# RohanVKashyap/resolution-pde

Measured on AMD Instinct MI355X. Metric: training samples/sec, FFNO2D NS 256^2, higher is better.
Workload: dtype f32; 1 GPU; FFNO2D(1,1,width=64,n_layers=4,n_modes=20,factor=4,ff_weight_norm,n_ff_layers=3,layer_norm,dropout=0.1) train step on [B,1,256,256] Gaussian random fields (BASELINE configs[2]); batch_per_gpu=32, global_batch=32, optimizer=AdamW lr=1e-3 (rpde.optim.FlatAdamW: torch.optim.AdamW's rule, one kernel), parallelism=single, grad_bucket_bytes=6828576, target=input advanced by a fixed spectral filter (utils/synthetic.py:advance)

## Files before the change

include/rpde.h:

```cpp
#ifndef RPDE_H
#define RPDE_H

#include <stddef.h>
#include <stdint.h>

#ifdef __cplusplus
extern "C" {
#endif

typedef enum {
  RPDE_OK = 0,
  RPDE_ERR_ARG = -1,
  RPDE_ERR_HIP = -2,
  RPDE_ERR_WORKSPACE = -3,
  RPDE_ERR_MODES = -4
} rpde_status;

enum { RPDE_NORM_BACKWARD = 0, RPDE_NORM_ORTHO = 1, RPDE_NORM_FORWARD = 2 };
enum { RPDE_MODE_FULL = 0, RPDE_MODE_LOWPASS = 1 };
enum { RPDE_ACT_IDENTITY = 0, RPDE_ACT_GELU = 1, RPDE_ACT_RELU = 2 };
enum { RPDE_EPI_MULAUX = 100 };

const char* rpde_last_error(void);
int rpde_version(void);
// ... 44 lines not shown
int rpde_fspectral1d_bwd(const float* grad_out, const float* spec_in, const float* w,
                         float* grad_x, float* grad_w, const float* grad_skip,
                         int B, int n, int C, int K, int mode, int norm,
                         void* ws, size_t ws_bytes, void* stream);

size_t rpde_fspectral2d_ws_bytes(int B, int M, int N, int C, int K);
size_t rpde_fspectral2d_spec_elems(int B, int M, int N, int C, int K, int axis );
int rpde_fspectral2d_fwd(const float* x, const float* w_y, const float* w_x, float* out,
                         float* spec_y, float* spec_x,
                         int B, int M, int N, int C, int K, int mode,
                         void* ws, size_t ws_bytes, void* stream);
int rpde_fspectral2d_bwd(const float* grad_out, const float* spec_y, const float* spec_x,
                         const float* w_y, const float* w_x,
                         float* grad_x, float* grad_wy, float* grad_wx, const float* grad_skip,
                         int B, int M, int N, int C, int K, int mode,
                         void* ws, size_t ws_bytes, void* stream);
size_t rpde_fspectral2d_prep_bytes(int M, int N, int C, int K);
size_t rpde_fspectral2d_eval_ws_bytes(int B, int M, int N, int C, int K);
int rpde_fspectral2d_prepare(const float* w_y, const float* w_x, int M, int N, int C, int K,
                             void* prep, size_t prep_bytes, void* stream);
int rpde_fspectral2d_fwd_prepared(const float* x, const void* prep, float* out, int B, int M, int N, int C, int K,
                                  void* ws, size_t ws_bytes, void* stream);

size_t rpde_spectral1d_ws_bytes(int B, int Cin, int Cout, int n, int K);
int rpde_spectral1d_fwd(const float* x, const float* w, float* out, float* spec_in,
                        int B, int Cin, int Cout, int n, int K, int act_in,
                        void* ws, size_t ws_bytes, void* stream);
int rpde_spectral1d_bwd(const float* grad_out, const float* spec_in, const float* w,
                        const float* x, float* grad_x, float* grad_w,
                        int B, int Cin, int Cout, int n, int K, int act_in,
                        void* ws, size_t ws_bytes, void* stream);

size_t rpde_spectral2d_ws_bytes(int B, int Cin, int Cout, int M, int N, int m1, int m2);
size_t rpde_spectral2d_spec_elems(int B, int Cin, int M, int N, int m1, int m2);
int rpde_spectral2d_fwd(const float* x, const float* w1, const float* w2, float* out, float* spec_in,
                        int B, int Cin, int Cout, int M, int N, int m1, int m2, int act_in,
                        void* ws, size_t ws_bytes, void* stream);
int rpde_spectral2d_bwd(const float* grad_out, const float* spec_in, const float* w1, const float* w2,
                        const float* x, float* grad_x, float* grad_w1, float* grad_w2,
                        int B, int Cin, int Cout, int M, int N, int m1, int m2, int act_in,
                        void* ws, size_t ws_bytes, void* stream);

typedef struct {
  int n_layers; int dim; int factor;
  int layer_norm; float ln_eps;
  float dropout_p; uint64_t seed;
// ... 266 lines not shown
```

resolution-pde_amd/csrc/ff_fused.hip:

```cpp
#include "ff_fused.h"
#include "cw.h"
#include "h2.h"
#include "pointwise.h"

namespace rpde {

#ifdef RPDE_STAMPS
__device__ unsigned long long g_ffstamps[3 * 64];
#define FFSTAMP(i) do { if (stamp_on && stamp_t < 8) g_ffstamps[stamp_w * 64 + stamp_t * 8 + (i)] = __builtin_amdgcn_s_memtime(); } while (0)
__device__ unsigned long long g_fbstamps[3 * 64];
#define FBSTAMP(i) do { if (stamp_on && stamp_t >= 0 && stamp_t < 8) g_fbstamps[stamp_w * 64 + stamp_t * 8 + (i)] = __builtin_amdgcn_s_memtime(); } while (0)
#else
#define FFSTAMP(i) do { } while (0)
#define FBSTAMP(i) do { } while (0)
#endif

constexpr int FF_WAVES = 8;
constexpr int FF_FRAGS = 24;
constexpr int FF_IMG_BYTES = FF_WAVES * FF_FRAGS * 2048;
constexpr int FF_NCONST = 16;
constexpr int FF_PREP_BLOCKS = FF_WAVES * FF_FRAGS * 64 / 1024;

__global__ __launch_bounds__(1024) void k_ff3_prep(const float* __restrict__ w1, const float* __restrict__ w2,
                                                   const float* __restrict__ w3, const float* __restrict__ b1,
// ... 394 lines not shown
    for (int k = 0; k < 64; ++k) wv2[k] = w2[(64 * part + k) * 256 + col];
#pragma unroll
    for (int k = 0; k < 64; ++k) b += fabsf(wv2[k]);
    colp[0][part][col] = a; colp[1][part][col] = b;
    __syncthreads();
    if (tid < 256) {
      r3 = (colp[0][0][tid] + colp[0][1][tid]) + (colp[0][2][tid] + colp[0][3][tid]);
      r2 = (colp[1][0][tid] + colp[1][1][tid]) + (colp[1][2][tid] + colp[1][3][tid]);
    }
  }
  float v[5] = {m1, m2, m3, r3, r2};
#pragma unroll
  for (int k = 0; k < 5; ++k) { v[k] = wave_max(v[k]); if (l == 0) red[k][wv] = v[k]; }
  __syncthreads();
  if (tid < 5) { float a = 0.f; for (int i = 0; i < 16; ++i) a = fmaxf(a, red[tid][i]); fin[tid] = a; }
  __syncthreads();
  float sc[3], iv[3];
#pragma unroll
  for (int k = 0; k < 3; ++k) h2_scale(fin[k], 0, sc[k], iv[k]);
  if (tid == 0 && blockIdx.x == 0) { consts[0] = iv[0]; consts[1] = iv[1]; consts[2] = iv[2]; consts[3] = fin[3]; consts[4] = fin[4]; }
  for (int it = blockIdx.x * 1024 + tid; it < FF_WAVES * FF_FRAGS * 64; it += gridDim.x * 1024) {
    const int ln = it & 63, f = (it >> 6) % FF_FRAGS, w = it / (64 * FF_FRAGS);
    const int g = ln >> 4, li = ln & 15;
    float x[8];
    if (f < 4) {
      const int hid = 16 * (2 * w + (f >> 1)) + li;
#pragma unroll
      for (int j = 0; j < 8; ++j) x[j] = w3[(32 * (f & 1) + frag_perm(g, j)) * 256 + hid] * sc[2];
    } else if (f < 20) {
      const int hid1 = 16 * (2 * w + ((f - 4) >> 3)) + li, kap = (f - 4) & 7;
#pragma unroll
      for (int j = 0; j < 8; ++j) x[j] = w2[(32 * kap + frag_perm(g, j)) * 256 + hid1] * sc[1];
    } else {
      const int feat = 16 * (f - 20) + li;
#pragma unroll
      for (int j = 0; j < 8; ++j) x[j] = w1[(32 * w + frag_perm(g, j)) * 64 + feat] * sc[0];
    }
    h2_put_frag(img + ((long)(w * FF_FRAGS + f)) * 2048 + ln * 16, x);
  }
}

constexpr int FFB_PART = 704;
struct FF3B {
  const float* g; const float* z3; const float* d1; const float* d2;
  float* dz3; float* du2; float* du1; float* dx;
  const char* wimg; const float* consts;
  const float* gamma; const float* beta;
  float* part;
  long P; int layer_norm; float eps; int post_act;
  DropCfg drop2;
  DropCfg drop0, drop1;
  float dmax;
  int ntiles;
};

constexpr int FB_DZBUF = 0;
constexpr int FB_DUBUF = FB_DZBUF + 8192;
constexpr int FB_W3L = FB_DUBUF + 32768;
constexpr int FB_D2 = FB_W3L + 32768;
// ... 410 lines not shown
```

resolution-pde_amd/csrc/fspectral.hip:

```cpp
#include "rpde_internal.h"
#include "plan.h"
#include "pointwise.h"
#include "fused_spectral.h"
#include "mix1d.h"

namespace rpde {

struct Axis {
  int n;
  int keff, kp;
  int rows;
  int zdiv;
  long s1, s2;
  long ld;
  const rpde_plan* plan;
};

static inline int split_for(long k_total, int tiles) {
  long s = 512 / (tiles > 0 ? tiles : 1);
  const long cap = (k_total + 127) / 128;
  if (s > cap) s = cap;
  if (s < 1) s = 1;
  if (s > 512) s = 512;
  return (int)s;
}

static int dft_analysis(const Axis& ax, const float* field, float* spec, int C, bool adjoint_of_synthesis, hipStream_t st) {
// ... 297 lines not shown
  RPDE_CARVE("fspectral1d_fwd", AxisFwdWork, wk, ws, ws_bytes, ax, C, mode, mix1d_ok(B, C));
  hipStream_t st = as_stream(stream);
  RPDE_TRY(make_axis(ax, n, K, norm, B, 1, (long)n * C, 0, C, st));
  return axis_fwd(ax, x, w, K, out, spec_in, C, mode, 0, wk, st);
}

int rpde_fspectral1d_bwd(const float* grad_out, const float* spec_in, const float* w, float* grad_x, float* grad_w,
                         const float* grad_skip, int B, int n, int C, int K, int mode, int norm, void* ws, size_t ws_bytes,
                         void* stream) {
  RPDE_CHECK_ARG(grad_out && spec_in && B > 0 && n > 0 && C > 0 && K > 0, "fspectral1d_bwd: bad arguments");
  RPDE_CHECK_ARG(mode == RPDE_MODE_LOWPASS || w, "fspectral1d_bwd: null weight");
  Axis ax; axis_dims(ax, n, K, B);
  RPDE_CARVE("fspectral1d_bwd", AxisBwdWork, wk, ws, ws_bytes, ax, C, mode, mix1d_ok(B, C));
  hipStream_t st = as_stream(stream);
  RPDE_TRY(make_axis(ax, n, K, norm, B, 1, (long)n * C, 0, C, st));
  return axis_bwd(ax, grad_out, spec_in, w, K, grad_x, grad_w, C, mode, 0, wk, st, grad_skip);
}

size_t rpde_fspectral2d_ws_bytes(int B, int M, int N, int C, int K) {
  Axis ay, ax;
  axes2d_dims(ay, ax, B, M, N, K);
  const size_t n = ws_max(axis_ws_bytes(ay, C), axis_ws_bytes(ax, C));
  if (!fused2d_ok(M, N, C, ay.keff, ax.keff)) return n;
  return ws_max(n, ws_max(ws_measure<Fused2dFwdWork>(ay, ax, C), ws_measure<Fused2dBwdWork>(ay, ax, C)));
}
size_t rpde_fspectral2d_spec_elems(int B, int M, int N, int C, int K, int axis) {
  Axis ay, ax;
  axes2d_dims(ay, ax, B, M, N, K);
  const Axis& a = axis == 0 ? ay : ax;
  return spec_floats(a, C) + (fused2d_ok(M, N, C, ay.keff, ax.keff) ? (size_t)a.rows : 0);
}

int rpde_fspectral2d_fwd(const float* x, const float* w_y, const float* w_x, float* out, float* spec_y, float* spec_x, int B,
                         int M, int N, int C, int K, int mode, void* ws, size_t ws_bytes, void* stream) {
  RPDE_CHECK_ARG(x && out && spec_y && spec_x && B > 0 && M > 0 && N > 0 && C > 0 && K > 0, "fspectral2d_fwd: bad arguments");
  RPDE_CHECK_ARG(mode == RPDE_MODE_LOWPASS || (w_y && w_x), "fspectral2d_fwd: null weight");
  RPDE_CHECK_ARG(mode == RPDE_MODE_FULL || mode == RPDE_MODE_LOWPASS, "fspectral2d_fwd: mode %d", mode);
  hipStream_t st = as_stream(stream);
  Axis ay, ax;
  axes2d_dims(ay, ax, B, M, N, K);
  Arena ar(ws, ws_bytes);
  if (fused2d_ok(M, N, C, ay.keff, ax.keff)) {
    const Fused2dFwdWork wk(ar, ay, ax, C);
    RPDE_CLAIM_WS("fspectral2d_fwd", ar, ws_bytes);
    RPDE_TRY(make_axes2d(ay, ax, B, M, N, C, K, st));
    return fused2d_fwd(ay, ax, x, w_y, w_x, out, spec_y, spec_x, B, M, N, C, K, mode, wk, st);
  }
// ... 77 lines not shown
```

resolution-pde_amd/models/ffno.py:

```python
from __future__ import annotations

import numpy as np
import torch
import torch.nn as nn

from models.custom_layer import WNLinear
from models.spectral_convolution import FSpectralConv1d, FSpectralConv2d
from rpde import ops


def _coord(c, device):
    if not isinstance(c, torch.Tensor):
        c = torch.tensor(c, dtype=torch.float)
    return c.to(device=device, dtype=torch.float32).contiguous()


class FFNO1D(nn.Module):
    def __init__(self, in_channels, out_channels, width=64, n_layers=4, n_modes=16, factor=4, ff_weight_norm=False,
                 n_ff_layers=2, layer_norm=False, dropout=0.0, grid=None, mode="full", fft_norm="ortho",
                 activation="identity", use_grid=True):
        super().__init__()
        self.in_channels, self.out_channels, self.hidden_dim = in_channels, out_channels, width
        self.n_layers, self.n_modes, self.grid = n_layers, n_modes, grid
        self.use_grid = grid
# ... 33 lines not shown
        self.fourier_layers = nn.ModuleList([
            FSpectralConv2d(width, n_modes, factor=factor, ff_weight_norm=ff_weight_norm, n_ff_layers=n_ff_layers,
                            layer_norm=layer_norm, dropout=dropout, mode=mode)
            for _ in range(n_layers)])
        self.out_proj = WNLinear(width, out_channels, wnorm=True) if ff_weight_norm else nn.Linear(width, out_channels)

    def get_grid(self, shape, device):
        b, m, n = shape[0], shape[1], shape[2]
        if self.grid is not None:
            gx, gy = _coord(self.grid[0], device), _coord(self.grid[1], device)
        else:
            gx = torch.tensor(np.linspace(0, 1, m), dtype=torch.float).to(device)
            gy = torch.tensor(np.linspace(0, 1, n), dtype=torch.float).to(device)
        gx = gx.reshape(1, m, 1, 1).repeat([b, 1, n, 1])
        gy = gy.reshape(1, 1, n, 1).repeat([b, m, 1, 1])
        return torch.cat((gx, gy), dim=-1)

    @staticmethod
    def _apply_linear(mod, h):
        if isinstance(mod, WNLinear):
            return mod(h)
        return ops.linear(h, mod.weight, mod.bias)

    def forward(self, x):
        if self.use_grid:
            gx = gy = None
            if self.grid is not None:
                gx, gy = _coord(self.grid[0], x.device), _coord(self.grid[1], x.device)
            h = ops.concat_grid(x, 2, 0.0, 1.0, channels_last=True, gridx=gx, gridy=gy)
        else:
            h = ops.to_channels_last(x)
        h = self._apply_linear(self.in_proj, h)
        for layer in self.fourier_layers:
            h, _ = layer(h, residual=h)
        return ops.to_channels_first(self._apply_linear(self.out_proj, h))
```

resolution-pde_amd/models/spectral_convolution.py:

```python
from __future__ import annotations

import torch
import torch.nn as nn
from torch.nn import functional as F

from models.custom_layer import FeedForward
from rpde import ops

act_registry = {"gelu": F.gelu, "identity": nn.Identity(), "relu": F.relu}


class SpectralConv1d(nn.Module):

    def __init__(self, in_channels, out_channels, modes1):
        super().__init__()
        self.in_channels, self.out_channels, self.modes1 = in_channels, out_channels, modes1
        self.scale = 1 / (in_channels * out_channels)
        self.weights1 = nn.Parameter(self.scale * torch.rand(in_channels, out_channels, modes1, dtype=torch.cfloat))

    def forward(self, x, act_in="identity"):
        return ops.spectral1d(x, self.weights1, act_in)


class SpectralConv2d(nn.Module):
# ... 46 lines not shown
        return self.backcast_ff(x, residual=residual, post_act=self.activation), None


class FSpectralConv2d(nn.Module):

    def __init__(self, d_model, modes, forecast_ff=None, backcast_ff=None, fourier_weight=None, factor=4,
                 ff_weight_norm=False, n_ff_layers=2, layer_norm=False, use_fork=False, dropout=0.0, mode="full"):
        super().__init__()
        self.in_dim = self.out_dim = d_model
        self.n_modes, self.mode, self.use_fork = modes, mode, use_fork
        self.fourier_weight = fourier_weight if fourier_weight else _fourier_weights(d_model, modes, 2)
        self.backcast_ff = backcast_ff if backcast_ff else FeedForward(
            d_model, factor, n_layers=n_ff_layers, ff_weight_norm=ff_weight_norm, layer_norm=layer_norm, dropout=dropout)
        self.forecast_ff = forecast_ff
        if use_fork and not self.forecast_ff:
            self.forecast_ff = FeedForward(
                d_model, factor, n_layers=n_ff_layers, ff_weight_norm=ff_weight_norm, layer_norm=layer_norm,
                dropout=dropout)

    def forward_fourier(self, x, with_skip=False):
        return ops.fspectral2d(x, self.fourier_weight[0], self.fourier_weight[1], self.n_modes, self.mode,
                               with_skip=with_skip)

    def forward(self, x, batch_dt=None, residual=None):
        if self.mode != "no-fourier":
            if residual is x and torch.is_grad_enabled() and x.requires_grad:
                x, residual = self.forward_fourier(x, with_skip=True)
            else:
                x = self.forward_fourier(x)
        b = self.backcast_ff(x, residual=residual)
        f = self.forecast_ff(x) if self.use_fork else None
        return b, f
```

resolution-pde_amd/rpde/_lib.py:

```python
from __future__ import annotations

import ctypes as C
import os
from typing import Optional, Sequence

import torch

_HERE = os.path.dirname(os.path.abspath(__file__))
LIB_PATH = os.environ.get("RPDE_LIB") or os.path.join(_HERE, "lib", "librpde_hip.so")

ACT = {"identity": 0, "gelu": 1, "relu": 2}
NORM = {"backward": 0, "ortho": 1, "forward": 2}
MODE = {"full": 0, "low-pass": 1}

ERR_ARG, ERR_HIP, ERR_WORKSPACE, ERR_MODES = -1, -2, -3, -4


class RpdeError(RuntimeError):
    pass


class GemmDesc(C.Structure):
    _fields_ = [
        ("A", C.c_void_p), ("B", C.c_void_p), ("C", C.c_void_p),
# ... 44 lines not shown
    "rpde_split_weights": (_I, [_P, _I, C.c_int64, _I, _I, _P, _P]),
    "rpde_fspectral1d_ws_bytes": (_Z, [_I, _I, _I, _I]),
    "rpde_fspectral1d_spec_elems": (_Z, [_I, _I, _I, _I]),
    "rpde_fspectral1d_fwd": (_I, [_P, _P, _P, _P, _I, _I, _I, _I, _I, _I, _P, _Z, _P]),
    "rpde_fspectral1d_bwd": (_I, [_P, _P, _P, _P, _P, _P, _I, _I, _I, _I, _I, _I, _P, _Z, _P]),
    "rpde_fspectral2d_ws_bytes": (_Z, [_I, _I, _I, _I, _I]),
    "rpde_fspectral2d_spec_elems": (_Z, [_I, _I, _I, _I, _I, _I]),
    "rpde_fspectral2d_fwd": (_I, [_P, _P, _P, _P, _P, _P, _I, _I, _I, _I, _I, _I, _P, _Z, _P]),
    "rpde_fspectral2d_bwd": (_I, [_P, _P, _P, _P, _P, _P, _P, _P, _P, _I, _I, _I, _I, _I, _I, _P, _Z, _P]),
    "rpde_spectral1d_ws_bytes": (_Z, [_I, _I, _I, _I, _I]),
    "rpde_spectral1d_fwd": (_I, [_P, _P, _P, _P, _I, _I, _I, _I, _I, _I, _P, _Z, _P]),
    "rpde_spectral1d_bwd": (_I, [_P, _P, _P, _P, _P, _P, _I, _I, _I, _I, _I, _I, _P, _Z, _P]),
    "rpde_spectral2d_ws_bytes": (_Z, [_I, _I, _I, _I, _I, _I, _I]),
    "rpde_spectral2d_spec_elems": (_Z, [_I, _I, _I, _I, _I, _I]),
    "rpde_spectral2d_fwd": (_I, [_P, _P, _P, _P, _P, _I, _I, _I, _I, _I, _I, _I, _I, _P, _Z, _P]),
    "rpde_spectral2d_bwd": (_I, [_P, _P, _P, _P, _P, _P, _P, _P, _I, _I, _I, _I, _I, _I, _I, _I, _P, _Z, _P]),
    "rpde_feedforward_ws_bytes": (_Z, [_L, _I, _I, _I]),
    "rpde_feedforward_fwd_ws_bytes": (_Z, [_I, _I, _I]),
    "rpde_feedforward_is_fused": (_I, [_I, _I, _I, _L]),
    "rpde_feedforward_fwd": (_I, [C.POINTER(FFParams), _P, _P, _PP, _PP, _P, _P, _L, _P, _Z, _P]),
    "rpde_feedforward_bwd": (_I, [C.POINTER(FFParams), _P, _PP, _PP, _P, _P, _P, _PP, _PP, _P, _P, _L, _P, _Z, _P]),
    "rpde_feedforward_prepare": (_I, [C.POINTER(FFParams), _P, _Z, _P]),
    "rpde_feedforward_fwd_prepared": (_I, [C.POINTER(FFParams), _P, _P, _P, _L, _P, _Z, _P]),
    "rpde_fspectral2d_prep_bytes": (_Z, [_I, _I, _I, _I]),
    "rpde_fspectral2d_eval_ws_bytes": (_Z, [_I, _I, _I, _I, _I]),
    "rpde_fspectral2d_prepare": (_I, [_P, _P, _I, _I, _I, _I, _P, _Z, _P]),
    "rpde_fspectral2d_fwd_prepared": (_I, [_P, _P, _P, _I, _I, _I, _I, _I, _P, _Z, _P]),
    "rpde_fno2d_lift_block_eval_ws_bytes": (_Z, [_I] * 7),
    "rpde_fno2d_lift_block_eval_ok": (_I, [_I] * 7),
    "rpde_fno2d_lift_block_eval_fwd": (_I, [_P] * 10 + [_I] * 8 + [_P, _Z, _P]),
    "rpde_linear_ws_bytes": (_Z, [_L, _I, _I]),
    "rpde_weight_norm_fwd": (_I, [_P, _P, _P, _I, _I, _P]),
    "rpde_weight_norm_bwd": (_I, [_P, _P, _P, _P, _P, _I, _I, _P]),
    "rpde_linear_fwd": (_I, [_P, _P, _P, _P, _L, _I, _I, _P]),
    "rpde_linear_bwd": (_I, [_P, _P, _P, _P, _P, _P, _L, _I, _I, _P, _Z, _P]),
    "rpde_conv1x1_ws_bytes": (_Z, [_I, _I, _I, _L]),
    "rpde_conv1x1_fwd": (_I, [_P, _P, _P, _P, _I, _I, _I, _L, _I, _I, _P]),
    "rpde_conv1x1_act_fwd": (_I, [_P, _P, _P, _P, _I, _I, _I, _L, _I, _I, _I, _P]),
    "rpde_fnoblock2d_eval_ws_bytes": (_Z, [_I, _I, _I, _I, _I, _I, _I]),
    "rpde_fnoblock2d_eval_ok": (_I, [_I, _I, _I, _I, _I]),
    "rpde_fnoblock2d_eval_fwd": (_I, [_P, _P, _P, _P, _P, _P, _I, _I, _I, _I, _I, _I, _I, _I, _P, _Z, _P]),
    "rpde_fnoblock2d_proj_eval_ok": (_I, [_I, _I, _I, _I, _I, _I, _I, _I]),
    "rpde_fnoblock2d_proj_eval_fwd": (_I, [_P, _P, _P, _P, _P, _P, _P, _P, _P, _P, _I, _I, _I, _I, _I, _I, _I, _I, _I, _I, _P, _Z, _P]),
    "rpde_conv_mlp_ok": (_I, [_I, _I, _I, _L]),
    "rpde_conv_mlp_fwd": (_I, [_P, _P, _P, _P, _P, _P, _I, _I, _I, _I, _L, _I, _P]),
    "rpde_conv1x1_bwd": (_I, [_P, _P, _P, _P, _P, _P, _I, _I, _I, _L, _I, _I, _P, _Z, _P]),
# ... 157 lines not shown
```

resolution-pde_amd/rpde/ops.py:

```python
from __future__ import annotations

import contextlib
import os

import ctypes as C
from typing import Callable, List, NamedTuple, Optional, Sequence, Tuple

import torch

from . import _lib
from ._lib import ACT, MODE, NORM, check, load, ptr, ptr_array, run, stream_ptr, workspace


def _f32c(t: torch.Tensor) -> torch.Tensor:
    if t.dtype != torch.float32:
        t = t.float()
    return t if t.is_contiguous() else t.contiguous()


def _as_float_storage(w: torch.Tensor) -> torch.Tensor:
    w = w if w.is_contiguous() else w.contiguous()
    return torch.view_as_real(w) if w.is_complex() else w


# ... 124 lines not shown
    if prep is None:
        return None
    out = torch.empty_like(x)
    run("fspectral2d_fwd_prepared", lib.rpde_fspectral2d_eval_ws_bytes(B, M, N, Cc, modes), x.device, ptr(x),
        prep.data_ptr(), ptr(out), B, M, N, Cc, modes)
    return out


def fspectral1d(x, w, modes: int, mode: str = "full", norm: str = "ortho", with_skip: bool = False):
    if mode not in MODE:
        raise ValueError(f"Mode {mode} not recognized")
    return _FSpectral1d.apply(x, w if mode == "full" else None, int(modes), MODE[mode], NORM[norm], bool(with_skip))


def fspectral2d(x, wy, wx, modes: int, mode: str = "full", with_skip: bool = False):
    if mode not in MODE:
        return (torch.zeros_like(x), x) if with_skip else torch.zeros_like(x)
    full = mode == "full"
    if full and _FROZEN is not None and not torch.is_grad_enabled() and x.is_cuda:
        out = _fspectral2d_frozen(x, wy, wx, int(modes))
        if out is not None:
            return (out, x) if with_skip else out
    return _FSpectral2d.apply(x, wy if full else None, wx if full else None, int(modes), MODE[mode], bool(with_skip))


_DROP_EPOCH: dict = {}


def drop_epoch(device) -> torch.Tensor:
    dev = torch.device(device)
    key = (dev.type, dev.index if dev.index is not None else torch.cuda.current_device())
    t = _DROP_EPOCH.get(key)
    if t is None:
        t = torch.zeros(1, dtype=torch.int64, device=dev)
        _DROP_EPOCH[key] = t
    return t


class _FeedForward(torch.autograd.Function):
    @staticmethod
    def forward(ctx, x, residual, cfg, *params):
        lib = load()
        L, dim, factor, layer_norm, eps, p_drop, seed, post_act, grad_on = cfg
        shape = x.shape
        x2 = _f32c(x).reshape(-1, dim)
        P = x2.shape[0]
# ... 1441 lines not shown
```

Baseline: 1010 samples/s.

## Fold input lift into first Fourier layer's spectral analysis on low-channel input

Because the lift is a linear map from a few input channels (Cin up to 4), the first layer's factorized spectral transform can be computed on the raw input u and mixed with w_in·w_fourier premultiplied weights. This skips running the analysis FFT over 64 lifted channels. The backward pass reduces gradients through small per-mode tables instead of full spectra. The change also drops the unused w1 fragment preparation in the feedforward prep kernel. It adds several new kernels and a special path that applies only when the input does not require grad.

```diff
diff --git a/include/rpde.h b/include/rpde.h
--- a/include/rpde.h
+++ b/include/rpde.h
@@ -90,6 +90,17 @@
 int rpde_fspectral2d_fwd_prepared(const float* x, const void* prep, float* out, int B, int M, int N, int C, int K,
                                   void* ws, size_t ws_bytes, void* stream);
 
+int rpde_lifted_fspectral2d_ok(int M, int N, int C, int Cin, int K);
+size_t rpde_lifted_fspectral2d_spec_elems(int B, int M, int N, int Cin, int K);
+int rpde_lifted_fspectral2d_fwd(const float* u, const float* w_in, const float* b_in, const float* w_y, const float* w_x,
+                                float* out, float* spec_u, int B, int M, int N, int C, int Cin, int K,
+                                void* ws, size_t ws_bytes, void* stream);
+int rpde_lifted_fspectral2d_bwd(const float* grad_out, const float* spec_u, const float* w_in, const float* b_in,
+                                const float* w_y, const float* w_x,
+                                float* grad_w_in, float* grad_b_in, float* grad_wy, float* grad_wx,
+                                int B, int M, int N, int C, int Cin, int K,
+                                void* ws, size_t ws_bytes, void* stream);
+
 size_t rpde_spectral1d_ws_bytes(int B, int Cin, int Cout, int n, int K);
 int rpde_spectral1d_fwd(const float* x, const float* w, float* out, float* spec_in,
                         int B, int Cin, int Cout, int n, int K, int act_in,
diff --git a/resolution-pde_amd/csrc/ff_fused.hip b/resolution-pde_amd/csrc/ff_fused.hip
--- a/resolution-pde_amd/csrc/ff_fused.hip
+++ b/resolution-pde_amd/csrc/ff_fused.hip
@@ -440,19 +440,16 @@
   for (int it = blockIdx.x * 1024 + tid; it < FF_WAVES * FF_FRAGS * 64; it += gridDim.x * 1024) {
     const int ln = it & 63, f = (it >> 6) % FF_FRAGS, w = it / (64 * FF_FRAGS);
     const int g = ln >> 4, li = ln & 15;
+    if (f >= 20) continue;
     float x[8];
     if (f < 4) {
       const int hid = 16 * (2 * w + (f >> 1)) + li;
 #pragma unroll
       for (int j = 0; j < 8; ++j) x[j] = w3[(32 * (f & 1) + frag_perm(g, j)) * 256 + hid] * sc[2];
-    } else if (f < 20) {
+    } else {
       const int hid1 = 16 * (2 * w + ((f - 4) >> 3)) + li, kap = (f - 4) & 7;
 #pragma unroll
       for (int j = 0; j < 8; ++j) x[j] = w2[(32 * kap + frag_perm(g, j)) * 256 + hid1] * sc[1];
-    } else {
-      const int feat = 16 * (f - 20) + li;
-#pragma unroll
-      for (int j = 0; j < 8; ++j) x[j] = w1[(32 * w + frag_perm(g, j)) * 64 + feat] * sc[0];
     }
     h2_put_frag(img + ((long)(w * FF_FRAGS + f)) * 2048 + ln * 16, x);
   }
diff --git a/resolution-pde_amd/csrc/fspectral.hip b/resolution-pde_amd/csrc/fspectral.hip
--- a/resolution-pde_amd/csrc/fspectral.hip
+++ b/resolution-pde_amd/csrc/fspectral.hip
@@ -3,6 +3,7 @@
 #include "pointwise.h"
 #include "fused_spectral.h"
 #include "mix1d.h"
+#include "lifted_spectral.h"
 
 namespace rpde {
 
@@ -346,7 +347,8 @@
   axes2d_dims(ay, ax, B, M, N, K);
   const size_t n = ws_max(axis_ws_bytes(ay, C), axis_ws_bytes(ax, C));
   if (!fused2d_ok(M, N, C, ay.keff, ax.keff)) return n;
-  return ws_max(n, ws_max(ws_measure<Fused2dFwdWork>(ay, ax, C), ws_measure<Fused2dBwdWork>(ay, ax, C)));
+  return ws_max(ws_max(n, lifted2d_ws_bytes(B, M, N, K)),
+                ws_max(ws_measure<Fused2dFwdWork>(ay, ax, C), ws_measure<Fused2dBwdWork>(ay, ax, C)));
 }
 size_t rpde_fspectral2d_spec_elems(int B, int M, int N, int C, int K, int axis) {
   Axis ay, ax;
diff --git a/resolution-pde_amd/csrc/lifted_spectral.h b/resolution-pde_amd/csrc/lifted_spectral.h
--- /dev/null
+++ b/resolution-pde_amd/csrc/lifted_spectral.h
@@ -0,0 +1,9 @@
+#pragma once
+#include <cstddef>
+
+namespace rpde {
+
+constexpr int LIFT_MAXC = 4;
+size_t lifted2d_ws_bytes(int B, int M, int N, int K);
+
+}
diff --git a/resolution-pde_amd/csrc/lifted_spectral.hip b/resolution-pde_amd/csrc/lifted_spectral.hip
--- /dev/null
+++ b/resolution-pde_amd/csrc/lifted_spectral.hip
@@ -0,0 +1,510 @@
+#include "fused_spectral.h"
+#include "h2.h"
+#include "lifted_spectral.h"
+#include "workspace.h"
+
+namespace rpde {
+
+constexpr int LIFT_LT = 32;
+constexpr int LIFT_ML = 16;
+
+struct LiftGeom {
+  int B, M, N, keff, kp, R;
+  long lines[2];
+  int n[2];
+};
+
+static LiftGeom lift_geom(int B, int M, int N, int K) {
+  LiftGeom g;
+  g.B = B; g.M = M; g.N = N;
+  const int ky = K < N / 2 + 1 ? K : N / 2 + 1;
+  g.keff = ky; g.kp = r4(ky); g.R = 2 * g.kp;
+  g.lines[0] = (long)B * M; g.lines[1] = (long)B * N;
+  g.n[0] = N; g.n[1] = M;
+  return g;
+}
+
+template <int CIN>
+__global__ __launch_bounds__(256) void k_lift_analysis(const float* __restrict__ u, const float* __restrict__ fa_y,
+                                                       const float* __restrict__ fa_x, int ldn_y, int ldn_x,
+                                                       float* __restrict__ s_y, float* __restrict__ s_x, int B, int M, int N, int R,
+                                                       int nblk_y) {
+  constexpr int LS = 32 * CIN + 4;
+  constexpr int TS = 36;
+  constexpr int NU = 32 * 32 * CIN / 256, NT = 6;
+  __shared__ __attribute__((aligned(16))) float tab[48 * TS];
+  __shared__ __attribute__((aligned(16))) float tile[LIFT_LT * LS];
+  const int tid = threadIdx.x;
+  const int a = blockIdx.x >= nblk_y ? 1 : 0;
+  const long l0 = (long)(a ? blockIdx.x - nblk_y : blockIdx.x) * LIFT_LT;
+  const int n = a ? M : N;
+  const float* __restrict__ fa = a ? fa_x : fa_y;
+  const int ldn = a ? ldn_x : ldn_y;
+  const int line = tid >> 3, rg = tid & 7, NI = R / 8;
+  float acc[6][CIN];
+#pragma unroll
+  for (int i = 0; i < 6; ++i)
+#pragma unroll
+    for (int c = 0; c < CIN; ++c) acc[i][c] = 0.f;
+  const long b = a ? l0 / N : l0 / M;
+  const long r0 = a ? l0 % N : l0 % M;
+  float ru[NU], rt[NT];
+  auto fetch = [&](int y0) {
+#pragma unroll
+    for (int v = 0; v < NU; ++v) {
+      const int e = tid + 256 * v, o = e / (32 * CIN), rem = e % (32 * CIN);
+      ru[v] = !a ? u[((b * M + r0 + o) * N + y0) * CIN + rem]
+                 : u[((b * M + y0 + o) * N + r0) * CIN + rem];
+    }
+#pragma unroll
+    for (int v = 0; v < NT; ++v) {
+      const int e = tid + 256 * v;
+      rt[v] = e < 32 * R ? fa[(long)(e >> 5) * ldn + y0 + (e & 31)] : 0.f;
+    }
+  };
+  fetch(0);
+  for (int y0 = 0; y0 < n; y0 += 32) {
+    __syncthreads();
+#pragma unroll
+    for (int v = 0; v < NU; ++v) {
+      const int e = tid + 256 * v, o = e / (32 * CIN), rem = e % (32 * CIN);
+      if (!a) tile[o * LS + rem] = ru[v];
+      else tile[(rem / CIN) * LS + o * CIN + rem % CIN] = ru[v];
+    }
+#pragma unroll
+    for (int v = 0; v < NT; ++v) {
+      const int e = tid + 256 * v;
+      if (e < 32 * R) tab[(e >> 5) * TS + (e & 31)] = rt[v];
+    }
+    __syncthreads();
+    if (y0 + 32 < n) fetch(y0 + 32);
+#pragma unroll 2
+    for (int q = 0; q < 8; ++q) {
+      float uv[4 * CIN];
+#pragma unroll
+      for (int c = 0; c < CIN; ++c) {
+        const float4 v = *reinterpret_cast<const float4*>(tile + line * LS + q * 4 * CIN + 4 * c);
+        uv[4 * c] = v.x; uv[4 * c + 1] = v.y; uv[4 * c + 2] = v.z; uv[4 * c + 3] = v.w;
+      }
+#pragma unroll
+      for (int i = 0; i < 6; ++i)
+        if (i < NI) {
+          const float4 t = *reinterpret_cast<const float4*>(tab + (rg + 8 * i) * TS + 4 * q);
+          const float tv[4] = {t.x, t.y, t.z, t.w};
+#pragma unroll
+          for (int yy = 0; yy < 4; ++yy)
+#pragma unroll
+            for (int c = 0; c < CIN; ++c) acc[i][c] = fmaf(tv[yy], uv[yy * CIN + c], acc[i][c]);
+        }
+    }
+  }
+  float* __restrict__ s = (a ? s_x : s_y) + (l0 + line) * (long)R * CIN;
+#pragma unroll
+  for (int i = 0; i < 6; ++i)
+    if (i < NI) {
+#pragma unroll
+      for (int c = 0; c < CIN; ++c) s[(rg + 8 * i) * CIN + c] = acc[i][c];
+    }
+}
+
+template <int CIN>
+__global__ __launch_bounds__(256) void k_lift_wprime(const float* __restrict__ w_in, const float* __restrict__ b_in,
+                                                     const float* __restrict__ w_y, const float* __restrict__ w_x, int K, int keff,
+                                                     int kp, float* __restrict__ wp) {
+  constexpr int CA = CIN + 1;
+  __shared__ float red[4][2 * CA][64];
+  const int k = blockIdx.x, a = blockIdx.y, o = threadIdx.x & 63, q = threadIdx.x >> 6;
+  const float* __restrict__ w = a ? w_x : w_y;
+  float re[CA], im[CA];
+#pragma unroll
+  for (int j = 0; j < CA; ++j) re[j] = im[j] = 0.f;
+  if (k < keff) {
+#pragma unroll 16
+    for (int i = 16 * q; i < 16 * q + 16; ++i) {
+      const float2 v = *reinterpret_cast<const float2*>(w + ((long)(i * 64 + o) * K + k) * 2);
+#pragma unroll
+      for (int j = 0; j < CA; ++j) {
+        const float t = j < CIN ? w_in[i * CIN + j] : (b_in ? b_in[i] : 0.f);
+        re[j] = fmaf(t, v.x, re[j]);
+        im[j] = fmaf(t, v.y, im[j]);
+      }
+    }
+  }
+#pragma unroll
+  for (int j = 0; j < CA; ++j) { red[q][2 * j][o] = re[j]; red[q][2 * j + 1][o] = im[j]; }
+  __syncthreads();
+  if (q == 0) {
+#pragma unroll
+    for (int j = 0; j < CA; ++j)
+      *reinterpret_cast<float2*>(wp + ((((long)a * kp + k) * CA + j) * 64 + o) * 2) =
+          make_float2((red[0][2 * j][o] + red[1][2 * j][o]) + (red[2][2 * j][o] + red[3][2 * j][o]),
+                      (red[0][2 * j + 1][o] + red[1][2 * j + 1][o]) + (red[2][2 * j + 1][o] + red[3][2 * j + 1][o]));
+  }
+}
+
+struct LiftMixP {
+  const float* s[2]; char* img[2]; float* inv[2];
+  const float* wp;
+  long nblk_y;
+  float sqn[2];
+  int kp, R;
+};
+
+template <int K32, int TG, int CIN>
+__global__ __launch_bounds__(256) void k_lift_mix(const LiftMixP P) {
+  constexpr int NF = K32 + (TG ? 1 : 0);
+  constexpr int CA = CIN + 1;
+  constexpr int BB = h2_block_bytes(K32, TG);
+  __shared__ float sl[LIFT_ML * 48 * CIN];
+  __shared__ float wmax[2][4];
+  const int tid = threadIdx.x, l = tid & 63, cb = tid >> 6, g = l >> 4, li = l & 15;
+  const int a = (long)blockIdx.x >= P.nblk_y ? 1 : 0;
+  const long line0 = ((long)blockIdx.x - (a ? P.nblk_y : 0)) * LIFT_ML;
+  const int R = P.R, o = 16 * cb + li;
+  const float sqn = P.sqn[a];
+  float2 wq[NF][4][CA];
+#pragma unroll
+  for (int s = 0; s < NF; ++s)
+#pragma unroll
+    for (int jj = 0; jj < 4; ++jj) {
+      const int k = 16 * s + 4 * g + jj;
+#pragma unroll
+      for (int j = 0; j < CA; ++j)
+        wq[s][jj][j] = k < P.kp ? *reinterpret_cast<const float2*>(P.wp + ((((long)a * P.kp + k) * CA + j) * 64 + o) * 2)
+                                : make_float2(0.f, 0.f);
+    }
+  {
+    const float* __restrict__ src = P.s[a] + line0 * (long)R * CIN;
+    for (int e = tid; e < LIFT_ML * R * CIN; e += 256) sl[e] = src[e];
+  }
+  __syncthreads();
+  for (int t = 0; t < LIFT_ML; ++t) {
+    const long line = line0 + t;
+    const float* __restrict__ sp = sl + t * R * CIN;
+    float v[NF][8];
+    float m = 0.f;
+#pragma unroll
+    for (int s = 0; s < NF; ++s)
+#pragma unroll
+      for (int jj = 0; jj < 4; ++jj) {
+        const int k = 16 * s + 4 * g + jj;
+        float re = 0.f, im = 0.f;
+        if (k < P.kp) {
+#pragma unroll
+          for (int j = 0; j < CIN; ++j) {
+            const float sr = sp[(2 * k) * CIN + j], si = sp[(2 * k + 1) * CIN + j];
+            const float2 w = wq[s][jj][j];
+            re = fmaf(sr, w.x, re); re = fmaf(-si, w.y, re);
+            im = fmaf(sr, w.y, im); im = fmaf(si, w.x, im);
+          }
+          if (k == 0) { re = fmaf(sqn, wq[s][jj][CIN].x, re); im = fmaf(sqn, wq[s][jj][CIN].y, im); }
+        }
+        v[s][2 * jj] = re; v[s][2 * jj + 1] = im;
+        m = fmaxf(m, fmaxf(fabsf(re), fabsf(im)));
+      }
+    m = wave_max(m);
+    if (l == 0) wmax[t & 1][cb] = m;
+    __syncthreads();
+    m = fmaxf(fmaxf(wmax[t & 1][0], wmax[t & 1][1]), fmaxf(wmax[t & 1][2], wmax[t & 1][3]));
+    float scale, inv;
+    h2_scale(m, H2_TABLE_EXP, scale, inv);
+    if (tid == 0) P.inv[a][line] = inv;
+    char* blk = P.img[a] + (line * 4 + cb) * (long)BB;
+#pragma unroll
+    for (int s = 0; s < NF; ++s) {
+#pragma unroll
+      for (int j = 0; j < 8; ++j) v[s][j] *= scale;
+      uint4 hi, lo;
+      h2_split8(v[s], hi, lo);
+      if (s < K32) {
+        *reinterpret_cast<uint4*>(blk + s * 1024 + l * 16) = hi;
+        *reinterpret_cast<uint4*>(blk + (K32 + s) * 1024 + l * 16) = lo;
+      } else if (g < TG) {
+#pragma unroll
+        for (int tt = 0; tt < 3; ++tt) {
+          const int slot = tt * TG + g;
+          *reinterpret_cast<uint4*>(blk + (2 * K32 + slot / 4) * 1024 + ((slot & 3) * 16 + li) * 16) = tt == 1 ? lo : hi;
+        }
+      }
+    }
+    if (TG > 0 && g == 0) {
+#pragma unroll
+      for (int slot = 3 * TG; slot < 4 * h2_np(TG); ++slot)
+        *reinterpret_cast<uint4*>(blk + (2 * K32 + slot / 4) * 1024 + ((slot & 3) * 16 + li) * 16) = make_uint4(0, 0, 0, 0);
+    }
+  }
+}
+
+template <int CIN>
+__global__ __launch_bounds__(512) void k_lift_tgrad(const float* __restrict__ g_y, const float* __restrict__ g_x,
+                                                    const float* __restrict__ s_y, const float* __restrict__ s_x, long lines_y,
+                                                    long lines_x, int kp, float sqn_y, float sqn_x, int S, float* __restrict__ part) {
+  constexpr int CA = CIN + 1;
+  const int o = threadIdx.x & 63, kg = __builtin_amdgcn_readfirstlane(threadIdx.x >> 6);
+  const int slab = blockIdx.x, a = blockIdx.y, R = 2 * kp;
+  const long lines = a ? lines_x : lines_y;
+  const float* __restrict__ G = a ? g_x : g_y;
+  const float* __restrict__ Su = a ? s_x : s_y;
+  const long lps = (lines + S - 1) / S, t0 = slab * lps, t1 = min(t0 + lps, lines);
+  float tre[3][CA], tim[3][CA];
+#pragma unroll
+  for (int i = 0; i < 3; ++i)
+#pragma unroll
+    for (int j = 0; j < CA; ++j) tre[i][j] = tim[i][j] = 0.f;
+  for (long t = t0; t < t1; t += 2) {
+    const bool two = t + 1 < t1;
+    float gre[2][3], gim[2][3];
+#pragma unroll
+    for (int h = 0; h < 2; ++h) {
+      const float* __restrict__ gl = G + (t + h) * (long)R * 64 + o;
+#pragma unroll
+      for (int i = 0; i < 3; ++i) {
+        const int k = kg + 8 * i;
+        const bool on = k < kp && (h == 0 || two);
+        gre[h][i] = on ? gl[(2 * k) * 64] : 0.f;
+        gim[h][i] = on ? gl[(2 * k + 1) * 64] : 0.f;
+      }
+    }
+#pragma unroll
+    for (int h = 0; h < 2; ++h) {
+      if (h == 1 && !two) break;
+      const float* __restrict__ sp = Su + (t + h) * (long)R * CIN;
+#pragma unroll
+      for (int i = 0; i < 3; ++i) {
+        const int k = kg + 8 * i;
+        if (k < kp) {
+#pragma unroll
+          for (int j = 0; j < CIN; ++j) {
+            const float sr = sp[(2 * k) * CIN + j], si = sp[(2 * k + 1) * CIN + j];
+            tre[i][j] = fmaf(sr, gre[h][i], tre[i][j]); tre[i][j] = fmaf(si, gim[h][i], tre[i][j]);
+            tim[i][j] = fmaf(sr, gim[h][i], tim[i][j]); tim[i][j] = fmaf(-si, gre[h][i], tim[i][j]);
+          }
+          tre[i][CIN] += gre[h][i]; tim[i][CIN] += gim[h][i];
+        }
+      }
+    }
+  }
+  const float sqn = a ? sqn_x : sqn_y;
+#pragma unroll
+  for (int i = 0; i < 3; ++i) {
+    const int k = kg + 8 * i;
+    if (k < kp) {
+      float* __restrict__ dst = part + ((((long)slab * 2 + a) * kp + k) * CA) * 128 + o * 2;
+#pragma unroll
+      for (int j = 0; j < CA; ++j) {
+        const float f = j < CIN ? 1.f : (k == 0 ? sqn : 0.f);
+        *reinterpret_cast<float2*>(dst + j * 128) = make_float2(tre[i][j] * f, tim[i][j] * f);
+      }
+    }
+  }
+}
+
+__global__ __launch_bounds__(1024) void k_lift_tfold(const float* __restrict__ part, float* __restrict__ T, long n_out, int S) {
+  __shared__ float red[16][64];
+  const int q = threadIdx.x >> 6, c = threadIdx.x & 63;
+  const long e = (long)blockIdx.x * 64 + c;
+  const int per = (S + 15) / 16, s0 = q * per, s1 = min(s0 + per, S);
+  float acc = 0.f;
+  if (e < n_out) {
+#pragma unroll 8
+    for (int s = s0; s < s1; ++s) acc += part[(long)s * n_out + e];
+  }
+  red[q][c] = acc;
+  __syncthreads();
+  for (int h = 8; h >= 1; h >>= 1) {
+    if (q < h) red[q][c] += red[q + h][c];
+    __syncthreads();
+  }
+  if (q == 0 && e < n_out) T[e] = red[0][c];
+}
+
+template <int CIN>
+__global__ __launch_bounds__(256) void k_lift_chain_w(const float* __restrict__ T, const float* __restrict__ w_in,
+                                                      const float* __restrict__ b_in, float* __restrict__ gw_y,
+                                                      float* __restrict__ gw_x, int K, int keff, int kp) {
+  constexpr int CA = CIN + 1;
+  const long idx = (long)blockIdx.x * 256 + threadIdx.x;
+  const int a = blockIdx.y;
+  float* __restrict__ gw = a ? gw_x : gw_y;
+  if (idx >= 4096L * K || !gw) return;
+  const int k = (int)(idx % K), o = (int)((idx / K) & 63), i = (int)(idx / K / 64);
+  float2 acc = make_float2(0.f, 0.f);
+  if (k < keff) {
+#pragma unroll
+    for (int j = 0; j < CA; ++j) {
+      const float t = j < CIN ? w_in[i * CIN + j] : (b_in ? b_in[i] : 0.f);
+      const float2 v = *reinterpret_cast<const float2*>(T + ((((long)a * kp + k) * CA + j) * 64 + o) * 2);
+      acc.x = fmaf(t, v.x, acc.x); acc.y = fmaf(t, v.y, acc.y);
+    }
+  }
+  *reinterpret_cast<float2*>(gw + idx * 2) = acc;
+}
+
+template <int CIN>
+__global__ __launch_bounds__(256) void k_lift_chain_in(const float* __restrict__ T, const float* __restrict__ w_y,
+                                                       const float* __restrict__ w_x, float* __restrict__ gw_in,
+                                                       float* __restrict__ gb_in, int K, int keff, int kp) {
+  constexpr int CA = CIN + 1;
+  __shared__ float red[CA][256];
+  const int i = blockIdx.x, tid = threadIdx.x;
+  float acc[CA];
+#pragma unroll
+  for (int j = 0; j < CA; ++j) acc[j] = 0.f;
+  for (int e = tid; e < 2 * keff * 64; e += 256) {
+    const int o = e & 63, k = (e >> 6) % keff, a = (e >> 6) / keff;
+    const float2 w = *reinterpret_cast<const float2*>((a ? w_x : w_y) + ((long)(i * 64 + o) * K + k) * 2);
+#pragma unroll
+    for (int j = 0; j < CA; ++j) {
+      const float2 v = *reinterpret_cast<const float2*>(T + ((((long)a * kp + k) * CA + j) * 64 + o) * 2);
+      acc[j] = fmaf(w.x, v.x, acc[j]); acc[j] = fmaf(w.y, v.y, acc[j]);
+    }
+  }
+#pragma unroll
+  for (int j = 0; j < CA; ++j) red[j][tid] = acc[j];
+  __syncthreads();
+  for (int h = 128; h >= 1; h >>= 1) {
+    if (tid < h) {
+#pragma unroll
+      for (int j = 0; j < CA; ++j) red[j][tid] += red[j][tid + h];
+    }
+    __syncthreads();
+  }
+  if (tid < CIN && gw_in) gw_in[i * CIN + tid] = red[tid][0];
+  if (tid == CIN && gb_in) gb_in[i] = red[CIN][0];
+}
+
+static int lift_slabs(const LiftGeom& g) {
+  const long fewest = g.lines[0] < g.lines[1] ? g.lines[0] : g.lines[1];
+  long S = fewest / 8;
+  if (S > 256) S = 256;
+  if (S < 1) S = 1;
+  return (int)S;
+}
+static size_t lift_t_floats(const LiftGeom& g, int Cin) { return (size_t)2 * g.kp * (Cin + 1) * 128; }
+static size_t lift_spec_floats(const LiftGeom& g, int Cin, int axis) { return (size_t)g.lines[axis] * g.R * Cin; }
+
+struct LiftFwdWork {
+  float* wp; void *imgy, *imgx; float *invy, *invx;
+  LiftFwdWork(Arena& ar, const LiftGeom& g, int Cin)
+      : wp(ar.take(lift_t_floats(g, Cin))), imgy(ar.take(fused2d_img_bytes(g.lines[0], g.R) / 4)),
+        imgx(ar.take(fused2d_img_bytes(g.lines[1], g.R) / 4)), invy(ar.take(g.lines[0])), invx(ar.take(g.lines[1])) {}
+};
+struct LiftBwdWork {
+  int S; float *gsy, *gsx, *part, *T;
+  LiftBwdWork(Arena& ar, const LiftGeom& g, int Cin)
+      : S(lift_slabs(g)), gsy(ar.take((size_t)g.lines[0] * g.R * 64)), gsx(ar.take((size_t)g.lines[1] * g.R * 64)),
+        part(ar.take((size_t)S * lift_t_floats(g, Cin))), T(ar.take(lift_t_floats(g, Cin))) {}
+};
+
+#define RPDE_LIFT_CIN(Cin, CALL)                  \
+  do {                                            \
+    switch (Cin) {                                \
+      case 1: { constexpr int CIN = 1; CALL; } break; \
+      case 2: { constexpr int CIN = 2; CALL; } break; \
+      case 3: { constexpr int CIN = 3; CALL; } break; \
+      default: { constexpr int CIN = 4; CALL; } break; \
+    }                                             \
+  } while (0)
+
+template <int CIN>
+static void launch_lift_mix(int R, dim3 grid, hipStream_t st, const LiftMixP& P) {
+  switch (R / 8) {
+    case 1: hipLaunchKernelGGL((k_lift_mix<0, 1, CIN>), grid, dim3(256), 0, st, P); break;
+    case 2: hipLaunchKernelGGL((k_lift_mix<0, 2, CIN>), grid, dim3(256), 0, st, P); break;
+    case 3: hipLaunchKernelGGL((k_lift_mix<0, 3, CIN>), grid, dim3(256), 0, st, P); break;
+    case 4: hipLaunchKernelGGL((k_lift_mix<1, 0, CIN>), grid, dim3(256), 0, st, P); break;
+    case 5: hipLaunchKernelGGL((k_lift_mix<1, 1, CIN>), grid, dim3(256), 0, st, P); break;
+    default: hipLaunchKernelGGL((k_lift_mix<1, 2, CIN>), grid, dim3(256), 0, st, P); break;
+  }
+}
+
+static int lift_plans(const LiftGeom& g, const rpde_plan** py, const rpde_plan** px, hipStream_t st) {
+  RPDE_TRY(get_plan(py, g.n[0], g.keff, RPDE_NORM_ORTHO, 0, PLAN_REAL, st));
+  return get_plan(px, g.n[1], g.keff, RPDE_NORM_ORTHO, 0, PLAN_REAL, st);
+}
+
+size_t lifted2d_ws_bytes(int B, int M, int N, int K) {
+  const LiftGeom g = lift_geom(B, M, N, K);
+  return ws_max(ws_measure<LiftFwdWork>(g, LIFT_MAXC), ws_measure<LiftBwdWork>(g, LIFT_MAXC));
+}
+
+}
+
+using namespace rpde;
+
+extern "C" {
+
+int rpde_lifted_fspectral2d_ok(int M, int N, int C, int Cin, int K) {
+  if (switch_off("RPDE_LIFTED_SPECTRAL") || M <= 0 || N <= 0 || K <= 0 || Cin < 1 || Cin > LIFT_MAXC) return 0;
+  const int ky = K < N / 2 + 1 ? K : N / 2 + 1, kx = K < M / 2 + 1 ? K : M / 2 + 1;
+  return fused2d_ok(M, N, C, ky, kx) ? 1 : 0;
+}
+
+size_t rpde_lifted_fspectral2d_spec_elems(int B, int M, int N, int Cin, int K) {
+  const LiftGeom g = lift_geom(B, M, N, K);
+  return lift_spec_floats(g, Cin, 0) + lift_spec_floats(g, Cin, 1);
+}
+
+int rpde_lifted_fspectral2d_fwd(const float* u, const float* w_in, const float* b_in, const float* w_y, const float* w_x,
+                                float* out, float* spec_u, int B, int M, int N, int C, int Cin, int K, void* ws,
+                                size_t ws_bytes, void* stream) {
+  RPDE_CHECK_ARG(u && w_in && w_y && w_x && out && spec_u && B > 0, "lifted_fspectral2d_fwd: bad arguments");
+  RPDE_CHECK_ARG(rpde_lifted_fspectral2d_ok(M, N, C, Cin, K), "lifted_fspectral2d_fwd: shape not on the lifted path");
+  const LiftGeom g = lift_geom(B, M, N, K);
+  RPDE_CARVE("lifted_fspectral2d_fwd", LiftFwdWork, wk, ws, ws_bytes, g, Cin);
+  hipStream_t st = as_stream(stream);
+  const rpde_plan *py, *px;
+  RPDE_TRY(lift_plans(g, &py, &px, st));
+  float* s_y = spec_u;
+  float* s_x = spec_u + lift_spec_floats(g, Cin, 0);
+  const int nby = (int)(g.lines[0] / LIFT_LT), nbx = (int)(g.lines[1] / LIFT_LT);
+  RPDE_LIFT_CIN(Cin, hipLaunchKernelGGL(k_lift_analysis<CIN>, dim3(nby + nbx), dim3(256), 0, st, u, py->fa, px->fa, py->ldn,
+                                        px->ldn, s_y, s_x, B, M, N, g.R, nby));
+  RPDE_LAUNCH_CHECK();
+  RPDE_LIFT_CIN(Cin, hipLaunchKernelGGL(k_lift_wprime<CIN>, dim3(g.kp, 2), dim3(256), 0, st, w_in, b_in, w_y, w_x, K, g.keff, g.kp,
+                                        wk.wp));
+  RPDE_LAUNCH_CHECK();
+  LiftMixP P;
+  P.s[0] = s_y; P.s[1] = s_x; P.img[0] = (char*)wk.imgy; P.img[1] = (char*)wk.imgx; P.inv[0] = wk.invy; P.inv[1] = wk.invx;
+  P.wp = wk.wp; P.nblk_y = g.lines[0] / LIFT_ML; P.sqn[0] = sqrtf((float)g.n[0]); P.sqn[1] = sqrtf((float)g.n[1]);
+  P.kp = g.kp; P.R = g.R;
+  const dim3 mgrid((unsigned)(g.lines[0] / LIFT_ML + g.lines[1] / LIFT_ML));
+  RPDE_LIFT_CIN(Cin, launch_lift_mix<CIN>(g.R, mgrid, st, P));
+  RPDE_LAUNCH_CHECK();
+  return fused2d_synthesis(wk.imgy, wk.imgx, wk.invy, wk.invx, py, px, 0, out, nullptr, B, M, N, st);
+}
+
+int rpde_lifted_fspectral2d_bwd(const float* grad_out, const float* spec_u, const float* w_in, const float* b_in,
+                                const float* w_y, const float* w_x, float* grad_w_in, float* grad_b_in, float* grad_wy,
+                                float* grad_wx, int B, int M, int N, int C, int Cin, int K, void* ws, size_t ws_bytes,
+                                void* stream) {
+  RPDE_CHECK_ARG(grad_out && spec_u && w_in && w_y && w_x && B > 0, "lifted_fspectral2d_bwd: bad arguments");
+  RPDE_CHECK_ARG(rpde_lifted_fspectral2d_ok(M, N, C, Cin, K), "lifted_fspectral2d_bwd: shape not on the lifted path");
+  const LiftGeom g = lift_geom(B, M, N, K);
+  RPDE_CARVE("lifted_fspectral2d_bwd", LiftBwdWork, wk, ws, ws_bytes, g, Cin);
+  hipStream_t st = as_stream(stream);
+  const rpde_plan *py, *px;
+  RPDE_TRY(lift_plans(g, &py, &px, st));
+  const float* s_y = spec_u;
+  const float* s_x = spec_u + lift_spec_floats(g, Cin, 0);
+  RPDE_TRY(fused2d_analysis(grad_out, wk.gsy, wk.gsx, nullptr, nullptr, py, px, 1, B, M, N, st));
+  RPDE_LIFT_CIN(Cin, hipLaunchKernelGGL(k_lift_tgrad<CIN>, dim3(wk.S, 2), dim3(512), 0, st, wk.gsy, wk.gsx, s_y, s_x, g.lines[0],
+                                        g.lines[1], g.kp, sqrtf((float)g.n[0]), sqrtf((float)g.n[1]), wk.S, wk.part));
+  RPDE_LAUNCH_CHECK();
+  const long n_out = (long)lift_t_floats(g, Cin);
+  hipLaunchKernelGGL(k_lift_tfold, dim3((unsigned)((n_out + 63) / 64)), dim3(1024), 0, st, wk.part, wk.T, n_out, wk.S);
+  RPDE_LAUNCH_CHECK();
+  if (grad_wy || grad_wx) {
+    RPDE_LIFT_CIN(Cin, hipLaunchKernelGGL(k_lift_chain_w<CIN>, dim3((unsigned)((4096L * K + 255) / 256), 2), dim3(256), 0, st, wk.T,
+                                          w_in, b_in, grad_wy, grad_wx, K, g.keff, g.kp));
+    RPDE_LAUNCH_CHECK();
+  }
+  if (grad_w_in || grad_b_in) {
+    RPDE_LIFT_CIN(Cin, hipLaunchKernelGGL(k_lift_chain_in<CIN>, dim3(64), dim3(256), 0, st, wk.T, w_y, w_x, grad_w_in, grad_b_in, K,
+                                          g.keff, g.kp));
+    RPDE_LAUNCH_CHECK();
+  }
+  return RPDE_OK;
+}
+
+}
diff --git a/resolution-pde_amd/models/ffno.py b/resolution-pde_amd/models/ffno.py
--- a/resolution-pde_amd/models/ffno.py
+++ b/resolution-pde_amd/models/ffno.py
@@ -79,6 +79,13 @@
             return mod(h)
         return ops.linear(h, mod.weight, mod.bias)
 
+    def _lifted_first_layer(self, u, w_in):
+        if len(self.fourier_layers) == 0 or self.fourier_layers[0].mode != "full":
+            return False
+        if not isinstance(self.in_proj, nn.Linear) or u.requires_grad:
+            return False
+        return ops.lifted_fspectral2d_ok(u, w_in, self.n_modes)
+
     def forward(self, x):
         if self.use_grid:
             gx = gy = None
@@ -87,7 +94,14 @@
             h = ops.concat_grid(x, 2, 0.0, 1.0, channels_last=True, gridx=gx, gridy=gy)
         else:
             h = ops.to_channels_last(x)
-        h = self._apply_linear(self.in_proj, h)
-        for layer in self.fourier_layers:
-            h, _ = layer(h, residual=h)
+        w_in = self.in_proj.effective_weight() if isinstance(self.in_proj, WNLinear) else self.in_proj.weight
+        u, h = h, ops.linear(h, w_in, self.in_proj.bias)
+        lifted = self._lifted_first_layer(u, w_in)
+        for i, layer in enumerate(self.fourier_layers):
+            if i == 0 and lifted:
+                fw = layer.fourier_weight
+                s = ops.lifted_fspectral2d(u, w_in, self.in_proj.bias, fw[0], fw[1], layer.n_modes)
+                h, _ = layer(h, residual=h, spectral=s)
+            else:
+                h, _ = layer(h, residual=h)
         return ops.to_channels_first(self._apply_linear(self.out_proj, h))
diff --git a/resolution-pde_amd/models/spectral_convolution.py b/resolution-pde_amd/models/spectral_convolution.py
--- a/resolution-pde_amd/models/spectral_convolution.py
+++ b/resolution-pde_amd/models/spectral_convolution.py
@@ -92,8 +92,10 @@
         return ops.fspectral2d(x, self.fourier_weight[0], self.fourier_weight[1], self.n_modes, self.mode,
                                with_skip=with_skip)
 
-    def forward(self, x, batch_dt=None, residual=None):
-        if self.mode != "no-fourier":
+    def forward(self, x, batch_dt=None, residual=None, spectral=None):
+        if spectral is not None:
+            x = spectral
+        elif self.mode != "no-fourier":
             if residual is x and torch.is_grad_enabled() and x.requires_grad:
                 x, residual = self.forward_fourier(x, with_skip=True)
             else:
diff --git a/resolution-pde_amd/rpde/_lib.py b/resolution-pde_amd/rpde/_lib.py
--- a/resolution-pde_amd/rpde/_lib.py
+++ b/resolution-pde_amd/rpde/_lib.py
@@ -90,6 +90,10 @@
     "rpde_feedforward_bwd": (_I, [C.POINTER(FFParams), _P, _PP, _PP, _P, _P, _P, _PP, _PP, _P, _P, _L, _P, _Z, _P]),
     "rpde_feedforward_prepare": (_I, [C.POINTER(FFParams), _P, _Z, _P]),
     "rpde_feedforward_fwd_prepared": (_I, [C.POINTER(FFParams), _P, _P, _P, _L, _P, _Z, _P]),
+    "rpde_lifted_fspectral2d_ok": (_I, [_I, _I, _I, _I, _I]),
+    "rpde_lifted_fspectral2d_spec_elems": (_Z, [_I, _I, _I, _I, _I]),
+    "rpde_lifted_fspectral2d_fwd": (_I, [_P] * 7 + [_I] * 6 + [_P, _Z, _P]),
+    "rpde_lifted_fspectral2d_bwd": (_I, [_P] * 10 + [_I] * 6 + [_P, _Z, _P]),
     "rpde_fspectral2d_prep_bytes": (_Z, [_I, _I, _I, _I]),
     "rpde_fspectral2d_eval_ws_bytes": (_Z, [_I, _I, _I, _I, _I]),
     "rpde_fspectral2d_prepare": (_I, [_P, _P, _I, _I, _I, _I, _P, _Z, _P]),
diff --git a/resolution-pde_amd/rpde/ops.py b/resolution-pde_amd/rpde/ops.py
--- a/resolution-pde_amd/rpde/ops.py
+++ b/resolution-pde_amd/rpde/ops.py
@@ -170,6 +170,54 @@
         if out is not None:
             return (out, x) if with_skip else out
     return _FSpectral2d.apply(x, wy if full else None, wx if full else None, int(modes), MODE[mode], bool(with_skip))
+
+
+class _LiftedFSpectral2d(torch.autograd.Function):
+
+    @staticmethod
+    def forward(ctx, u, w_in, b_in, wy, wx, modes: int):
+        lib = load()
+        u, w_in, wyf, wxf = _f32c(u), _f32c(w_in), _f32c(wy), _f32c(wx)
+        b_in = _f32c(b_in) if b_in is not None else None
+        B, M, N, Cin = u.shape
+        Cc = w_in.shape[0]
+        out = torch.empty(B, M, N, Cc, dtype=torch.float32, device=u.device)
+        spec = torch.empty(lib.rpde_lifted_fspectral2d_spec_elems(B, M, N, Cin, modes), dtype=torch.float32, device=u.device)
+        run("lifted_fspectral2d_fwd", lib.rpde_fspectral2d_ws_bytes(B, M, N, Cc, modes), u.device, ptr(u), ptr(w_in),
+            ptr(b_in), ptr(wyf), ptr(wxf), ptr(out), ptr(spec), B, M, N, Cc, Cin, modes)
+        ctx.save_for_backward(spec, w_in, wyf, wxf, *(() if b_in is None else (b_in,)))
+        ctx.dims = (B, M, N, Cc, Cin, modes)
+        return out
+
+    @staticmethod
+    def backward(ctx, g):
+        lib = load()
+        B, M, N, Cc, Cin, modes = ctx.dims
+        spec, w_in, wyf, wxf, *rest = ctx.saved_tensors
+        b_in = rest[0] if rest else None
+        g = _f32c(g)
+        need_in, need_b = ctx.needs_input_grad[1], b_in is not None and ctx.needs_input_grad[2]
+        need_w = ctx.needs_input_grad[3] or ctx.needs_input_grad[4]
+        gw_in = torch.empty_like(w_in) if need_in else None
+        gb_in = torch.empty_like(b_in) if need_b else None
+        gwy = torch.empty_like(wyf) if need_w else None
+        gwx = torch.empty_like(wxf) if need_w else None
+        run("lifted_fspectral2d_bwd", lib.rpde_fspectral2d_ws_bytes(B, M, N, Cc, modes), g.device, ptr(g), ptr(spec),
+            ptr(w_in), ptr(b_in), ptr(wyf), ptr(wxf), ptr(gw_in), ptr(gb_in), ptr(gwy), ptr(gwx), B, M, N, Cc, Cin, modes)
+        return None, gw_in, gb_in, gwy, gwx, None
+
+
+def lifted_fspectral2d_ok(u, w_in, modes: int) -> bool:
+    if not (u.is_cuda and u.dim() == 4 and u.dtype == torch.float32 and w_in.dtype == torch.float32):
+        return False
+    if not torch.is_grad_enabled():
+        return False
+    _, M, N, Cin = u.shape
+    return bool(load().rpde_lifted_fspectral2d_ok(M, N, w_in.shape[0], Cin, int(modes)))
+
+
+def lifted_fspectral2d(u, w_in, b_in, wy, wx, modes: int):
+    return _LiftedFSpectral2d.apply(u, w_in, b_in, wy, wx, int(modes))
 
 
 _DROP_EPOCH: dict = {}
```

Result: faster. 1031 samples/s (median of 6 runs) (+2.1%).
